# jizongFox/Self-paced-Contrastive-Learning

Measured on AMD Instinct MI355X. Metric: pretrain slices/sec/node (UNet+InfoNCE, 224^2, bs=32/GPU), higher is better.
Workload: dtype bf16; 1 GPU; BASELINE.json configs[1]: self-paced pretrain step, UNet base (max_channel=256) encoder to Conv5 + ProjectionHead(256,256,256) + SelfPacedSupConLoss(soft, partition labels, correct_grad) fwd+bwd + RAdam; slices_per_gpu=32, images_per_gpu_step=64, image=1x224x224, global_batch=32, parallelism=dp1, params=1311056, hipgraph=epocher, capture_steps=3

## Files before the change

include/spcl_hip.h:

```cpp
#ifndef SPCL_HIP_H
#define SPCL_HIP_H
#include <stddef.h>
#include <stdint.h>
#ifdef __cplusplus
extern "C" {
#endif

#define SPCL_F32 0
#define SPCL_BF16 1

#define SPCL_OK 0
#define SPCL_EINVAL (-1)
#define SPCL_ELAUNCH (-2)
#define SPCL_EUNSUPPORTED (-3)

#define SPCL_ABI_VERSION 28
int spcl_abi_version(void);
const char* spcl_last_error(void);

size_t spcl_supcon_workspace_bytes(int n, int d);
int spcl_supcon_forward(const float* z1, const float* z2, const float* labels, const float* mask, int n, int d,
                        float temperature, int sp_mode, float gamma, int correct_grad, float* ws, float* out,
                        void* stream);
int spcl_supcon_backward(const float* labels, const float* mask, int n, int d, float temperature, int sp_mode,
                         float gamma, const float* ws_fwd, float* ws_bwd, const float* out_fwd,
                         const float* grad_out, float* dz1, float* dz2, void* stream);
size_t spcl_supcon_bwd_workspace_bytes(int n, int d);
int spcl_supcon_unit_gradient_block(int n, int d, size_t* offset_floats, int* row_pitch);
int spcl_supcon_forward_heads(int K, const float* z1, const float* z2, size_t z_stride, const float* labels, int n,
                              int d, float temperature, int sp_mode, const float* gammas, int correct_grad, float* ws,
                              size_t ws_stride, float* out, void* stream);
int spcl_supcon_rows_supported(int n, int d);
int spcl_supcon_forward_rows(int K, const float* o1, const float* o2, size_t o_stride, const float* labels, int n, int d,
                             float temperature, int sp_mode, const float* gammas, int correct_grad, float* ws,
                             size_t ws_stride, float* out, void* stream);
int spcl_supcon_backward_heads(int K, const float* labels, int n, int d, float temperature, int sp_mode,
                               const float* gammas, const float* ws_fwd, size_t ws_stride, float* ws_bwd,
                               size_t wsb_stride, const float* out_fwd, const float* grad_out, float* dz1, float* dz2,
                               size_t z_stride, void* stream);
int spcl_supcon_materialize(const float* labels, const float* mask, int n, int d, float temperature, int sp_mode,
                            float gamma, const float* ws_fwd, float* sim_logits, float* sim_exp, float* pos_mask,
                            float* neg_mask, float* sp_mask, void* stream);

size_t spcl_supcon_xpos_workspace_bytes(int n, int d);
int spcl_supcon_xpos_forward(const float* z1, const float* z2, const float* labels, const float* mask, int n, int d,
                             float temperature, float* ws, float* out, void* stream);
int spcl_supcon_xpos_backward(const float* z1, const float* z2, int n, int d, float temperature, const float* ws,
                              const float* grad_out, float* dz1, float* dz2, void* stream);

// ... 107 lines not shown
int spcl_l2norm_rows_forward(const float* x, size_t rows, int O, float* z, void* stream);
int spcl_l2norm_rows_backward(const float* x, const float* dz, size_t rows, int O, float* dx, void* stream);

int spcl_group_l2norm_temp_forward(const float* l, size_t rows, long ld, int S, int K, int normalize, float T, float* z,
                                   void* stream);
int spcl_group_l2norm_temp_backward(const float* l, const float* dz, size_t rows, long ld, int S, int K, int normalize, float T,
                                    float* dl, void* stream);

#define SPCL_WGRAD_BATCH_MAX 16
typedef struct spcl_wgrad_item {
  const void* x;
  const void* dy;
  const float* in_scale;
  const float* in_shift;
  float* dw_oihw;
  int N, H, W, Cin, CinS, Cout, CoutS, in_mode;
  const void* x2;
  int x_up2;
} spcl_wgrad_item;
int spcl_conv_wgrad_batched_supported(int dtype, int Cin, int CinS, int Cout, int CoutS, int in_mode);
size_t spcl_conv_wgrad_batched_workspace_bytes(const spcl_wgrad_item* items, int n);
int spcl_conv3x3_wgrad_batched(const spcl_wgrad_item* items, int n, int accumulate, float* partial, void* stream);

#define SPCL_WGRAD_TAILS_MAX 16
typedef struct spcl_wgrad_tail {
  const float* partial;
  float* dw;
  int kind;
  int nsplit, nblk_ci, nblk_co, CIB, COB, Cin, Cout;
} spcl_wgrad_tail;
int spcl_wgrad_tail_capture(spcl_wgrad_tail* slot);
int spcl_conv3x3_wgrad_batched_tails(const spcl_wgrad_item* items, int n, const spcl_wgrad_tail* tails, int ntails,
                                     int accumulate, float* partial, void* stream);
int spcl_bn_finalize(float* stats, int ntiles, int C, int CS, const float* gamma, const float* beta,
                     float momentum, float eps, float* running_mean, float* running_var,
                     int64_t* num_batches_tracked, float* mean, float* invstd, float* scale, float* shift,
                     void* stream);
int spcl_bn_eval_affine(int C, int CS, const float* gamma, const float* beta, const float* running_mean,
                        const float* running_var, float eps, float* mean, float* invstd, float* scale, float* shift,
                        void* stream);
#define SPCL_BN_EVAL_MAX 32
typedef struct {
  const float* gamma;
  const float* beta;
  const float* running_mean;
  const float* running_var;
  float* st;
  int C, CS;
  float eps;
} spcl_bn_eval_item;
int spcl_bn_eval_affine_multi(const spcl_bn_eval_item* items, int n, void* stream);

int spcl_bnrelu_pool_forward(const void* y, int dtype, int N, int H, int W, int CS, const float* scale,
                             const float* shift, void* act_out, void* pool_out, void* stream);
size_t spcl_bnrelu_bwd_workspace_bytes(int N, int H, int W, int CS);
int spcl_bnrelu_pool_backward(const void* y, const void* dact, const void* dpool, int dtype, int N, int H, int W,
                              int C, int CS, const float* mean, const float* invstd, const float* scale,
                              const float* shift, int training, float* ws, float* dgamma, float* dbeta, void* dy,
                              void* stream);
int spcl_bnrelu_up2_forward(const void* y, int dtype, int N, int H, int W, int CS, const float* scale, const float* shift,
                            void* up_out, void* stream);
int spcl_bnrelu_pool_forward_strided(const void* y, int dtype, int N, int H, int W, int CS, const float* scale,
                                     const float* shift, void* act_out, int act_stride, void* pool_out, void* stream);
int spcl_bnrelu_pool_backward_strided(const void* y, const void* dact, int dact_stride, const void* dpool, int dtype, int N,
                                      int H, int W, int C, int CS, const float* mean, const float* invstd,
                                      const float* scale, const float* shift, int training, float* ws, float* dgamma,
// ... 328 lines not shown
```

self-paced-contrastive-learning_amd/csrc/wgrad.hip:

```cpp
#include <stdlib.h>
#include <vector>
#include "conv_common.hpp"

namespace spcl {

constexpr int WG_TW = 16, WG_HW = WG_TW + 2;

struct WgradArgs {
  const void* x;
  const void* x2;
  int xsplit;
  int x_up2;
  const void* dy;
  const float* in_scale;
  const float* in_shift;
  float* partial;
  int N, H, W, CinS, CinK, CoutS, in_mode;
  int tilesX, tilesY, ntiles, nblk_ci, nblk_co;
  int dbuf;
  int xcd_remap;
  unsigned long long* stamps;
};

template <typename T> __device__ __forceinline__ u32x4 wg_bnrelu_chunk(u32x4 raw, const float* sc, const float* sh);
template <> __device__ __forceinline__ u32x4 wg_bnrelu_chunk<float>(u32x4 raw, const float* s, const float* b) {
  f32x4 v = __builtin_bit_cast(f32x4, raw);
#pragma unroll
  for (int e = 0; e < 4; ++e) v[e] = fmaxf(fmaf(s[e], v[e], b[e]), 0.f);
  return __builtin_bit_cast(u32x4, v);
}
template <> __device__ __forceinline__ u32x4 wg_bnrelu_chunk<bf16_t>(u32x4 raw, const float* s, const float* b) {
  u32x4 out;
#pragma unroll
// ... 56 lines not shown
  static __device__ __forceinline__ int lane_col(int lane) { return Frag<bf16_t>::lane_col(lane); }
  static __device__ __forceinline__ int lane_chan_bytes(int lane) { return Frag<bf16_t>::lane_chan_bytes(lane); }
  static __device__ __forceinline__ type load(unsigned a0, int off, int pix_bytes, int plane_bytes) {
    type f;
    f.h = Frag<bf16_t>::load(a0, off, pix_bytes);
    f.m = Frag<bf16_t>::load(a0 + plane_bytes, off, pix_bytes);
    f.l = Frag<bf16_t>::load(a0 + 2 * plane_bytes, off, pix_bytes);
    return f;
  }
  static __device__ __forceinline__ f32x4 mfma(const type& a, const type& b, f32x4 c) {
    c = __builtin_amdgcn_mfma_f32_16x16x32_bf16(a.l, b.h, c, 0, 0, 0);
    c = __builtin_amdgcn_mfma_f32_16x16x32_bf16(a.h, b.l, c, 0, 0, 0);
    c = __builtin_amdgcn_mfma_f32_16x16x32_bf16(a.m, b.m, c, 0, 0, 0);
    c = __builtin_amdgcn_mfma_f32_16x16x32_bf16(a.m, b.h, c, 0, 0, 0);
    c = __builtin_amdgcn_mfma_f32_16x16x32_bf16(a.h, b.m, c, 0, 0, 0);
    c = __builtin_amdgcn_mfma_f32_16x16x32_bf16(a.h, b.h, c, 0, 0, 0);
    return c;
  }
  static constexpr int row_pad(int pix_bytes, int row_bytes) { return Frag<bf16_t>::row_pad(pix_bytes, row_bytes); }
};

#ifndef SPCL_WGRAD_STAMPS_BUILD
#define SPCL_WGRAD_STAMPS_BUILD 0
#endif
__device__ __forceinline__ void store_split(unsigned char* p, int plane_bytes, u32x4 v) {
  const Split3 a = split3_pair(__uint_as_float(v[0]), __uint_as_float(v[1]));
  const Split3 b = split3_pair(__uint_as_float(v[2]), __uint_as_float(v[3]));
  *(uint2*)p = make_uint2(a.hi, b.hi);
  *(uint2*)(p + plane_bytes) = make_uint2(a.mid, b.mid);
  *(uint2*)(p + 2 * plane_bytes) = make_uint2(a.lo, b.lo);
}

template <typename T, int MI, int NJ, int TH, int NWV, int IM>
__global__ __launch_bounds__(64 * NWV, 2) void conv3x3_wgrad_kernel(WgradArgs a) {
  constexpr int NTHR = 64 * NWV;
  constexpr int EPC = Chunk<T>::EPC;
  constexpr int LSZ = Frag<T>::LSZ, NPL = Frag<T>::PLANES, LCH = EPC * LSZ;
  constexpr int CIB = 16 * MI, COB = 16 * NJ;
  constexpr int XS = CIB * LSZ, DS = COB * LSZ;
  constexpr int XCP = CIB / EPC, DCP = COB / EPC;
  constexpr int XRP = WG_HW * XS + Frag<T>::row_pad(XS, WG_HW * XS);
  constexpr int DRP = WG_TW * DS + Frag<T>::row_pad(DS, WG_TW * DS);
  constexpr int NHROWS = TH + 2;
  constexpr int XPLB = NHROWS * XRP, DPLB = TH * DRP;
  constexpr int X_BYTES = NPL * XPLB, D_BYTES = NPL * DPLB, BUF_BYTES = X_BYTES + D_BYTES;
  constexpr int KSTEPS = TH * WG_TW / Frag<T>::KPIX;
  constexpr int XPL = NTHR / XCP, XRPI = XPL / WG_HW, NX = (NHROWS + XRPI - 1) / XRPI;
  constexpr int DPL = NTHR / DCP, DRPI = DPL / WG_TW, ND = (TH + DRPI - 1) / DRPI;
  static_assert(XRPI >= 1 && DRPI >= 1, "channel block too wide for the staging map");
  extern __shared__ __attribute__((aligned(16))) unsigned char lds[];
  const unsigned lds_base = (unsigned)(uintptr_t)(unsigned char __attribute__((address_space(3)))*)lds;

  const int lane = threadIdx.x & 63, wave = threadIdx.x >> 6;
  const int blk = blockIdx.y;
  const int bci = blk / a.nblk_co, bco = blk - bci * a.nblk_co;
  const int ci0 = bci * CIB, co0 = bco * COB;
  const int xch = threadIdx.x % XCP, xpl = threadIdx.x / XCP;
  const int xhy0 = xpl / WG_HW, xhx = xpl - xhy0 * WG_HW;
  const bool xact = xpl < XRPI * WG_HW;
  const int dch = threadIdx.x % DCP, dpl = threadIdx.x / DCP;
  const int dry0 = dpl / WG_TW, dcol = dpl - dry0 * WG_TW;
  float sc[EPC], sh[EPC];
  const bool bn_x2 = IM == 1 && a.x2 != nullptr;
  const bool bn_this = IM == 1 && (!bn_x2 || ci0 + xch * EPC >= a.xsplit);
  if (IM == 1) {
    const int cc = bn_x2 ? (bn_this ? ci0 + xch * EPC - a.xsplit : 0) : ci0 + xch * EPC;
#pragma unroll
    for (int e = 0; e < EPC; e += 4) {
      *(f32x4*)&sc[e] = *(const f32x4*)(a.in_scale + cc + e);
      *(f32x4*)&sh[e] = *(const f32x4*)(a.in_shift + cc + e);
    }
  }

  constexpr int NUNITS = 9 * MI, UPW = (NUNITS + NWV - 1) / NWV;
  f32x4 acc[UPW][NJ];
  int uoff[UPW];
#pragma unroll
  for (int uu = 0; uu < UPW; ++uu) {
    int u = wave + NWV * uu;
    if (u >= NUNITS) u = NUNITS - 1;
    const int tap = u / MI, m = u - tap * MI;
    const int ky = tap / 3, kx = tap - 3 * ky;
    uoff[uu] = ky * XRP + kx * XS + m * 16 * LSZ;
#pragma unroll
    for (int j = 0; j < NJ; ++j) acc[uu][j] = (f32x4){0.f, 0.f, 0.f, 0.f};
  }
  const unsigned xlane = (unsigned)(Frag<T>::lane_row(lane) * XRP + Frag<T>::lane_col(lane) * XS +
// ... 99 lines not shown
    constexpr bool K32 = Frag<T>::KPIX == 32;
    constexpr bool SKIP_DUP = NUNITS % NWV != 0;
    const bool last_real = wave + NWV * (UPW - 1) < NUNITS;
    auto kpos_x = [&](int ks) { return (K32 ? 2 * ks : ks / 4) * XRP + (K32 ? 0 : 4 * (ks % 4)) * XS; };
    auto kpos_d = [&](int ks) { return (K32 ? 2 * ks : ks / 4) * DRP + (K32 ? 0 : 4 * (ks % 4)) * DS; };
    typename Frag<T>::type bf[NJ], bf_next[NJ], af, af_next;
#pragma unroll
    for (int j = 0; j < NJ; ++j) bf[j] = Frag<T>::load(da0, kpos_d(0) + j * 16 * LSZ, DS, DPLB);
    af = Frag<T>::load(xa0 + uoff[0], kpos_x(0), XS, XPLB);
#pragma unroll
    for (int ks = 0; ks < KSTEPS; ++ks) {
#pragma unroll
      for (int uu = 0; uu < UPW; ++uu) {
        if (uu + 1 < UPW) af_next = Frag<T>::load(xa0 + uoff[uu + 1], kpos_x(ks), XS, XPLB);
        else if (ks + 1 < KSTEPS) {
          af_next = Frag<T>::load(xa0 + uoff[0], kpos_x(ks + 1), XS, XPLB);
#pragma unroll
          for (int j = 0; j < NJ; ++j) bf_next[j] = Frag<T>::load(da0, kpos_d(ks + 1) + j * 16 * LSZ, DS, DPLB);
        }
        if (!(SKIP_DUP && uu == UPW - 1 && !last_real)) {
#pragma unroll
          for (int j = 0; j < NJ; ++j) acc[uu][j] = Frag<T>::mfma(af, bf[j], acc[uu][j]);
        }
        af = af_next;
      }
#pragma unroll
      for (int j = 0; j < NJ; ++j) bf[j] = bf_next[j];
    }
  };

  unsigned long long t_store = 0, t_bar = 0, t_issue = 0, t_comp = 0, t_first = 0, t_all = 0, ntl = 0;
  const bool stamp = SPCL_WGRAD_STAMPS_BUILD && a.stamps != nullptr;
  const unsigned long long c_begin = stamp ? __builtin_amdgcn_s_memtime() : 0;
  const int G = (int)gridDim.x;
  const int pos = (a.xcd_remap && (G & 7) == 0) ? (int)(blockIdx.x & 7) * (G >> 3) + (int)(blockIdx.x >> 3) : (int)blockIdx.x;
  int tile = pos;
  int buf = 0;
  if (tile < a.ntiles) load_tile(tile);
  if (stamp) t_first = __builtin_amdgcn_s_memtime() - c_begin;
  while (tile < a.ntiles) {
    const unsigned long long c0 = stamp ? __builtin_amdgcn_s_memtime() : 0;
    store_tile(buf);
    const unsigned long long c1 = stamp ? __builtin_amdgcn_s_memtime() : 0;
    __syncthreads();
    const unsigned long long c2 = stamp ? __builtin_amdgcn_s_memtime() : 0;
    const int next = tile + gridDim.x;
    if (next < a.ntiles) load_tile(next);
    const unsigned long long c3 = stamp ? __builtin_amdgcn_s_memtime() : 0;
    compute_tile(buf);
    if (stamp) {
      t_store += c1 - c0; t_bar += c2 - c1; t_issue += c3 - c2; t_comp += __builtin_amdgcn_s_memtime() - c3;
      ++ntl;
    }
    if (a.dbuf) buf ^= 1;
    else __syncthreads();
    tile = next;
  }
  if (stamp) t_all = __builtin_amdgcn_s_memtime() - c_begin;

  const int r16 = lane & 15, g = lane >> 4;
  float* out = a.partial + ((size_t)blockIdx.x * gridDim.y + blk) * (9 * CIB * COB);
#pragma unroll
  for (int uu = 0; uu < UPW; ++uu) {
    const int u = wave + NWV * uu;
    if (u < NUNITS) {
      const int tap = u / MI, m = u - tap * MI;
#pragma unroll
      for (int j = 0; j < NJ; ++j)
#pragma unroll
        for (int r = 0; r < 4; ++r)
          out[(tap * CIB + m * 16 + 4 * g + r) * COB + j * 16 + r16] = acc[uu][j][r];
    }
  }
  if (stamp && threadIdx.x == 0) {
    unsigned long long* o = a.stamps + ((size_t)blockIdx.x * gridDim.y + blk) * 8;
    o[0] = t_first; o[1] = t_store; o[2] = t_bar; o[3] = t_issue; o[4] = t_comp; o[5] = t_all;
    o[6] = __builtin_amdgcn_s_memtime() - c_begin; o[7] = ntl;
  }
}

template <int VEC>
__global__ __launch_bounds__(1024) void wgrad_reduce_kernel(const float* __restrict__ partial, int nsplit, int nblk_ci,
                                                            int nblk_co, int CIB, int COB, int Cin, int Cout,
                                                            float* __restrict__ dw) {
  __shared__ float red[16][64 * VEC];
  const int nwaves = blockDim.x >> 6;
  const int lane = threadIdx.x & 63, wave = threadIdx.x >> 6;
  const int slab = 9 * CIB * COB;
  const int inner = (blockIdx.x * 64 + lane) * VEC;
  const int blk = blockIdx.y;
  const size_t nblk = (size_t)nblk_ci * nblk_co;
  float s[VEC];
#pragma unroll
  for (int e = 0; e < VEC; ++e) s[e] = 0.f;
  if (inner < slab) {
    const float* src = partial + (size_t)blk * slab + inner;
    const size_t stride = nblk * slab;
#pragma unroll 8
    for (int p = wave; p < nsplit; p += nwaves) {
      if (VEC == 4) {
        const f32x4 v = *(const f32x4*)(src + (size_t)p * stride);
#pragma unroll
        for (int e = 0; e < VEC; ++e) s[e] += v[e];
      } else {
        s[0] += src[(size_t)p * stride];
      }
    }
  }
#pragma unroll
  for (int e = 0; e < VEC; ++e) red[wave][lane * VEC + e] = s[e];
// ... 211 lines not shown
  {
    const double px = (double)N * H * W, es = dtype == SPCL_F32 ? 4.0 : 2.0;
    prof_cost(px * ((in_mode == 2 ? CinS * 4.0 : CinK * es) + CoutS * es) + 9.0 * Cin * Cout * 4.0,
              2.0 * px * 9.0 * Cin * Cout);
  }
  if (dtype == SPCL_F32 && split) launch_wgrad_t<split_f32>(a, p, st);
  else if (dtype == SPCL_F32) launch_wgrad_t<float>(a, p, st);
  else if (dtype == SPCL_BF16) launch_wgrad_t<bf16_t>(a, p, st);
  else {
    set_error("conv3x3_wgrad: dtype %d", dtype);
    return SPCL_EINVAL;
  }
  if (tail != nullptr) {
    tail->partial = partial; tail->dw = dw_oihw; tail->kind = 0; tail->nsplit = p.nsplit; tail->nblk_ci = p.nblk_ci;
    tail->nblk_co = p.nblk_co; tail->CIB = 16 * p.MI; tail->COB = 16 * p.NJ; tail->Cin = Cin; tail->Cout = Cout;
  } else {
    launch_wgrad_reduce(partial, p.nsplit, p.nblk_ci, p.nblk_co, 16 * p.MI, 16 * p.NJ, Cin, Cout, dw_oihw, st);
  }
  if (a.stamps) {
    std::vector<unsigned long long> h(nwg * 8);
    (void)hipStreamSynchronize(st);
    (void)hipMemcpy(h.data(), a.stamps, h.size() * 8, hipMemcpyDeviceToHost);
    double s[8] = {0};
    for (size_t i = 0; i < nwg; ++i)
      for (int k = 0; k < 8; ++k) s[k] += (double)h[i * 8 + k];
    for (int k = 0; k < 8; ++k) s[k] /= (double)nwg;
    fprintf(stderr, "[wgrad stamps] %dx%d Cin%d Cout%d MI%d NJ%d TH%d wgs=%zu tiles/wg=%.1f | memtime ticks per wg: first-load "
            "issue %.0f, store %.0f, barrier %.0f, next-load issue %.0f, compute %.0f, loop total %.0f, with epilogue %.0f\n",
            H, W, Cin, Cout, p.MI, p.NJ, p.TH, nwg, s[7], s[0], s[1], s[2], s[3], s[4], s[5], s[6]);
  }
  SPCL_LAUNCH_CHECK("conv3x3_wgrad");
  return SPCL_OK;
}
```

self-paced-contrastive-learning_amd/functional.py:

```python
from __future__ import annotations

import ctypes
import math
import os
from ctypes import c_double, c_float, c_int

import torch

from . import native as _n

SP_NONE, SP_HARD, SP_SOFT = 0, 1, 2


def take_grad_sink(param, needed: bool = True):
    if not needed or param is None:
        return None
    sink = getattr(param, "_grad_sink", None)
    if sink is None or not getattr(param, "_grad_sink_armed", False):
        return None
    if sink.shape != param.shape or sink.dtype != torch.float32 or not sink.is_contiguous() or sink.device != param.device:
        return None
    param._grad_sink_armed = False
    return sink

# ... 1121 lines not shown
    if want_rows and stats_acc is None:
        nt = _n.call("spcl_conv_stat_rows", dt_code, N, H, W, cin_k, cout_s)
        rows = torch.empty(_n.call("spcl_bn_stats_elems", nt, cout_s), dtype=torch.float32, device=dev)
        rows.ntiles = nt
    _n.call("spcl_conv3x3_forward_acc", _n.ptr(x_store), dt_code, N, H, W, cin_k, cout_s, _n.ptr(wp),
            ctypes.byref(in_bn) if in_bn is not None else None, _n.ptr(in_scale), _n.ptr(in_shift), _n.ptr(y),
            _n.ptr(stats_acc), _n.ptr(rows), _n.stream())
    return y, rows


def _bn_stats(stats, cfg: BlockCfg, C, cs, gamma, beta, which, dev):
    st = torch.empty(4, cs, dtype=torch.float32, device=dev)
    g, b = gamma.detach().contiguous().float(), beta.detach().contiguous().float()
    rm, rv, nbt = cfg.buffers[which]
    if cfg.training:
        upd = cfg.track[which]
        _n.call("spcl_bn_finalize", _n.ptr(stats), stats.ntiles, C, cs, _n.ptr(g), _n.ptr(b), c_float(cfg.momentum),
                c_float(cfg.eps), _n.ptr(rm if upd else None), _n.ptr(rv if upd else None),
                _n.ptr(nbt if upd else None), _n.ptr(st[0]), _n.ptr(st[1]), _n.ptr(st[2]), _n.ptr(st[3]), _n.stream())
    else:
        pre = _EVAL_AFFINE.pop((rm.data_ptr(), cs), None) if rm.dtype == torch.float32 else None
        if pre is not None:
            return pre
        _n.call("spcl_bn_eval_affine", C, cs, _n.ptr(g), _n.ptr(b), _n.ptr(rm), _n.ptr(rv), c_float(cfg.eps),
                _n.ptr(st[0]), _n.ptr(st[1]), _n.ptr(st[2]), _n.ptr(st[3]), _n.stream())
    return st


class DeferredWgrads:

    def __init__(self):
        self.items, self.keep, self.targets = [], [], set()
        self.tails = []

    def add(self, x_store, dy, scale, shift, sink, N, H, W, cin, cin_s, cout, cout_s, in_mode, x2=None, x_up2=False):
        it = _n.WgradItem(x_store.data_ptr(), dy.data_ptr(), scale.data_ptr() if scale is not None else None,
                          shift.data_ptr() if shift is not None else None, sink.data_ptr(), N, H, W, cin, cin_s, cout,
                          cout_s, in_mode, x2.data_ptr() if x2 is not None else None, 1 if x_up2 else 0)
        self.items.append(it)
        self.keep.append((x_store, dy, scale, shift, x2))
        self.targets.add(sink.data_ptr())
        if len(self.items) == _QUEUE_MAX[0]:
            self.flush()

    def capture_tail(self, sink, keep, launch):
        tail = _n.WgradTail()
        _n.call("spcl_wgrad_tail_capture", ctypes.byref(tail))
        try:
            launch()
        finally:
            _n.call("spcl_wgrad_tail_capture", None)
        if tail.kind < 0:
            return False
        self.tails.append(tail)
        self.keep.append(keep)
        self.targets.add(sink.data_ptr())
        if len(self.tails) == _QUEUE_MAX[1]:
            self.flush()
        return True

    def flush(self):
        if not self.items and not self.tails:
            return
        wgrad_batched(self.items, accumulate=False, device=self.keep[0][1].device, tails=self.tails)
        self.items, self.keep, self.tails = [], [], []


_QUEUE_MAX = (min(_n.WGRAD_BATCH_MAX, int(os.environ.get("SPCL_WGRAD_QUEUE_MAX", _n.WGRAD_BATCH_MAX))),
              min(_n.WGRAD_TAILS_MAX, int(os.environ.get("SPCL_WGRAD_QUEUE_MAX", _n.WGRAD_TAILS_MAX))))
_CONV_UP2 = os.environ.get("SPCL_CONV_UP2", "1") != "0"
_UP2_BWD_FUSED = os.environ.get("SPCL_UP2_BWD_FUSED", "1") != "0"
_CONV_SPLIT = os.environ.get("SPCL_CONV_SPLIT", "1") != "0"
_CONV_CAT = os.environ.get("SPCL_CONV_CAT", "1") != "0"
_PACK_AT = os.environ.get("SPCL_PACK_AT", "1") != "0"
_ACC_FILL = os.environ.get("SPCL_ACC_FILL", "1") != "0"
_GAP = os.environ.get("SPCL_GAP", "1") != "0"
_TAILS = os.environ.get("SPCL_WGRAD_TAILS", "1") != "0"


def sink_queue(sink):
    return getattr(sink, "_spcl_queue", None) if sink is not None else None


def wgrad_batched(items, accumulate, device, tails=()):
    arr, ws = None, None
    if items:
        arr = (_n.WgradItem * len(items))(*items)
        nbytes = _n.call("spcl_conv_wgrad_batched_workspace_bytes", arr, len(items))
        if nbytes == 0:
            raise RuntimeError("wgrad_batched: unsupported item (bf16 NHWC, channel counts multiples of 64, in_mode 0/1)")
        ws = torch.empty(nbytes // 4, dtype=torch.float32, device=device)
    tarr = (_n.WgradTail * len(tails))(*tails) if tails else None
    _n.call("spcl_conv3x3_wgrad_batched_tails", arr, len(items), tarr, len(tails), int(bool(accumulate)), _n.ptr(ws),
            _n.stream())


def _wgrad(x_store, dy, dt_code, N, H, W, cin, cin_s, cin_k, cout, cout_s, in_mode, scale, shift, sink=None):
    dev = dy.device
    queue = sink_queue(sink)
    if (queue is not None and cin_s == cin_k
            and _n.call("spcl_conv_wgrad_batched_supported", dt_code, cin, cin_s, cout, cout_s, in_mode)):
        queue.add(x_store, dy, scale, shift, sink, N, H, W, cin, cin_s, cout, cout_s, in_mode)
        return None
    nbytes = _n.call("spcl_conv_wgrad_workspace_bytes", N, H, W, cin_k, cout_s)
    ws = torch.empty(nbytes // 4, dtype=torch.float32, device=dev)
    dw = _grad_buffer(sink, (cout, cin, 3, 3), dev)

    def launch():
        _n.call("spcl_conv3x3_wgrad", _n.ptr(x_store), _n.ptr(dy), dt_code, N, H, W, cin, cin_s, cin_k, cout, cout_s,
                in_mode, _n.ptr(scale), _n.ptr(shift), _n.ptr(ws), _n.ptr(dw), _n.stream())

    if queue is not None and _TAILS:
        if queue.capture_tail(sink, (ws, dy, x_store, scale, shift), launch):
            return None
        return dw
    launch()
    return dw


def _wgrad_up2(x_half, dy, dt_code, N, H, W, cin, cout, cout_s, sink=None):
    dev = dy.device
    queue = sink_queue(sink)
    if queue is not None and _n.call("spcl_conv_wgrad_batched_supported", dt_code, cin, cin, cout, cout_s, 0):
        queue.add(x_half, dy, None, None, sink, N, H, W, cin, cin, cout, cout_s, 0, x_up2=True)
        return None
    nbytes = _n.call("spcl_conv_wgrad_workspace_bytes", N, H, W, cin, cout_s)
    ws = torch.empty(nbytes // 4, dtype=torch.float32, device=dev)
    dw = _grad_buffer(sink, (cout, cin, 3, 3), dev)

    def launch():
        _n.call("spcl_conv3x3_wgrad_up2", _n.ptr(x_half), _n.ptr(dy), dt_code, N, H, W, cin, cout, cout_s, _n.ptr(ws),
                _n.ptr(dw), _n.stream())

    if queue is not None and _TAILS:
        if queue.capture_tail(sink, (ws, dy, x_half), launch):
# ... 2233 lines not shown
```

self-paced-contrastive-learning_amd/native.py:

```python
from __future__ import annotations

import ctypes
import os
from ctypes import c_char_p, c_double, c_float, c_int, c_long, c_size_t, c_void_p

import torch

HERE = os.path.dirname(os.path.abspath(__file__))
LIB_PATH = os.path.join(HERE, "lib", "libspcl_hip.so")
SPCL_F32, SPCL_BF16 = 0, 1

_lib = None

_P = c_void_p
_SIGNATURES = {
    "spcl_abi_version": (c_int, []),
    "spcl_last_error": (c_char_p, []),
    "spcl_supcon_workspace_bytes": (c_size_t, [c_int, c_int]),
    "spcl_supcon_forward": (c_int, [_P, _P, _P, _P, c_int, c_int, c_float, c_int, c_float, c_int, _P, _P, _P]),
    "spcl_supcon_backward": (c_int, [_P, _P, c_int, c_int, c_float, c_int, c_float, _P, _P, _P, _P, _P, _P, _P]),
    "spcl_supcon_bwd_workspace_bytes": (c_size_t, [c_int, c_int]),
    "spcl_supcon_unit_gradient_block": (c_int, [c_int, c_int, _P, _P]),
    "spcl_supcon_materialize": (c_int, [_P, _P, c_int, c_int, c_float, c_int, c_float, _P, _P, _P, _P, _P, _P, _P]),
    "spcl_supcon_xpos_workspace_bytes": (c_size_t, [c_int, c_int]),
# ... 31 lines not shown
    "spcl_conv_pack_weights_multi_zero": (c_int, [_P, c_int, c_int, _P, c_int, c_int, c_int, _P, _P, c_size_t, _P]),
    "spcl_conv_num_tiles": (c_int, [c_int, c_int, c_int]),
    "spcl_conv_stat_rows": (c_int, [c_int, c_int, c_int, c_int, c_int, c_int]),
    "spcl_conv_set_gemm": (None, [c_int]),
    "spcl_conv_set_f32_split": (None, [c_int]),
    "spcl_conv_get_f32_split": (c_int, []),
    "spcl_conv_cat_supported": (c_int, [c_int, c_int, c_int, c_int, c_int, c_int]),
    "spcl_conv3x3_forward_cat": (c_int, [_P, _P, c_int, c_int, c_int, c_int, c_int, c_int, _P, _P, _P, _P, _P, _P]),
    "spcl_conv_split_supported": (c_int, [c_int, c_int, c_int, c_int, c_int, c_int]),
    "spcl_conv3x3_forward_split": (c_int, [_P, c_int, c_int, c_int, c_int, c_int, c_int, _P, _P, _P, _P]),
    "spcl_conv_split_bnstats_supported": (c_int, [c_int, c_int, c_int, c_int, c_int, c_int]),
    "spcl_conv3x3_dgrad_split_bnstats": (c_int, [_P, c_int, c_int, c_int, c_int, c_int, c_int, _P, _P, _P, _P, _P, _P, _P, _P,
                                                 _P]),
    "spcl_conv_up2_supported": (c_int, [c_int, c_int, c_int, c_int, c_int, c_int]),
    "spcl_conv3x3_forward_up2": (c_int, [_P, c_int, c_int, c_int, c_int, c_int, c_int, _P, _P, _P, _P]),
    "spcl_conv3x3_wgrad_up2": (c_int, [_P, _P, c_int, c_int, c_int, c_int, c_int, c_int, c_int, _P, _P, _P]),
    "spcl_conv3x3_wgrad_cat": (c_int, [_P, _P, _P, c_int, c_int, c_int, c_int, c_int, c_int, c_int, _P, _P, _P, _P, _P]),
    "spcl_bn_stats_elems": (c_size_t, [c_int, c_int]),
    "spcl_conv3x3_forward": (c_int, [_P, c_int, c_int, c_int, c_int, c_int, c_int, c_int, _P, c_int, _P, _P, _P, _P,
                                     _P]),
    "spcl_supcon_forward_heads": (c_int, [c_int, _P, _P, c_size_t, _P, c_int, c_int, c_float, c_int, _P, c_int, _P,
                                          c_size_t, _P, _P]),
    "spcl_supcon_rows_supported": (c_int, [c_int, c_int]),
    "spcl_supcon_forward_rows": (c_int, [c_int, _P, _P, c_size_t, _P, c_int, c_int, c_float, c_int, _P, c_int, _P,
                                         c_size_t, _P, _P]),
    "spcl_supcon_backward_heads": (c_int, [c_int, _P, c_int, c_int, c_float, c_int, _P, _P, c_size_t, _P, c_size_t, _P,
                                           _P, _P, _P, c_size_t, _P]),
    "spcl_conv_wgrad_workspace_bytes": (c_size_t, [c_int, c_int, c_int, c_int, c_int]),
    "spcl_conv3x3_wgrad": (c_int, [_P, _P, c_int, c_int, c_int, c_int, c_int, c_int, c_int, c_int, c_int, c_int, _P,
                                   _P, _P, _P, _P]),
    "spcl_conv_wgrad_batched_supported": (c_int, [c_int, c_int, c_int, c_int, c_int, c_int]),
    "spcl_conv_wgrad_batched_workspace_bytes": (c_size_t, [_P, c_int]),
    "spcl_conv3x3_wgrad_batched": (c_int, [_P, c_int, c_int, _P, _P]),
    "spcl_wgrad_tail_capture": (c_int, [_P]),
    "spcl_conv3x3_wgrad_batched_tails": (c_int, [_P, c_int, _P, c_int, c_int, _P, _P]),
    "spcl_bn_finalize": (c_int, [_P, c_int, c_int, c_int, _P, _P, c_float, c_float, _P, _P, _P, _P, _P, _P, _P, _P]),
    "spcl_bn_eval_affine": (c_int, [c_int, c_int, _P, _P, _P, _P, c_float, _P, _P, _P, _P, _P]),
    "spcl_bn_eval_affine_multi": (c_int, [_P, c_int, _P]),
    "spcl_bnrelu_pool_forward": (c_int, [_P, c_int, c_int, c_int, c_int, c_int, _P, _P, _P, _P, _P]),
    "spcl_bnrelu_up2_forward": (c_int, [_P, c_int, c_int, c_int, c_int, c_int, _P, _P, _P, _P]),
    "spcl_bnrelu_pool_forward_strided": (c_int, [_P, c_int, c_int, c_int, c_int, c_int, _P, _P, _P, c_int, _P, _P]),
    "spcl_bnrelu_pool_backward_strided": (c_int, [_P, _P, c_int, _P, c_int, c_int, c_int, c_int, c_int, c_int, _P, _P, _P,
                                                  _P, c_int, _P, _P, _P, _P, _P]),
    "spcl_bnrelu_bwd_workspace_bytes": (c_size_t, [c_int, c_int, c_int, c_int]),
    "spcl_bnrelu_pool_backward": (c_int, [_P, _P, _P, c_int, c_int, c_int, c_int, c_int, c_int, _P, _P, _P, _P,
                                          c_int, _P, _P, _P, _P, _P]),
    "spcl_bnrelu_backward_up2": (c_int, [_P, _P, _P, c_int, c_int, c_int, c_int, c_int, c_int, _P, _P, _P, _P, c_int, _P, _P, _P, _P,
                                         _P]),
    "spcl_bnrelu_backward_bcast": (c_int, [_P, _P, c_int, c_int, c_int, c_int, c_int, c_int, _P, _P, _P, _P, c_int, _P, _P,
                                           _P, _P, _P]),
    "spcl_bnrelu_image_wgrad_workspace_bytes": (c_size_t, [c_int, c_int, c_int, c_int]),
    "spcl_bnrelu_backward_image_wgrad": (c_int, [_P, _P, _P, c_int, c_int, c_int, c_int, c_int, c_int, _P, _P, _P, _P,
                                                 c_int, _P, _P, _P, _P, _P]),
    "spcl_accumulate_scalars": (c_int, [c_int, _P, _P, _P, _P]),
    "spcl_stage_bytes": (c_int, [_P, _P, c_size_t, _P]),
    "spcl_conv_dgrad_bnstats_supported": (c_int, [c_int, c_int, c_int, c_int, c_int, c_int]),
    "spcl_conv3x3_dgrad_bnstats": (c_int, [_P, c_int, c_int, c_int, c_int, c_int, c_int, _P, _P, _P, _P, _P, _P, _P, _P]),
    "spcl_conv_dgrad_poolstats_supported": (c_int, [c_int, c_int, c_int, c_int, c_int, c_int, c_int, c_int]),
    "spcl_conv3x3_dgrad_poolstats": (c_int, [_P, c_int, c_int, c_int, c_int, c_int, c_int, _P, _P, _P, c_int, c_int, _P, _P,
                                             _P, _P, _P]),
    "spcl_bnrelu_pool_backward_rows": (c_int, [_P, _P, _P, c_int, c_int, c_int, c_int, c_int, c_int, c_int, _P, _P, _P, _P,
                                               c_int, _P, _P, _P, _P, _P]),
    "spcl_bnrelu_backward_rows": (c_int, [_P, _P, _P, _P, c_int, c_int, c_int, c_int, c_int, c_int, c_int, _P, _P, _P, _P,
                                          c_int, _P, _P, _P, _P, _P, _P]),
    "spcl_image_autocorr_rows": (c_int, [c_int, c_int, c_int]),
    "spcl_image_autocorr": (c_int, [_P, c_int, c_int, c_int, _P, _P]),
# ... 160 lines not shown
class WgradItem(ctypes.Structure):
    _fields_ = [("x", c_void_p), ("dy", c_void_p), ("in_scale", c_void_p), ("in_shift", c_void_p),
                ("dw_oihw", c_void_p), ("N", c_int), ("H", c_int), ("W", c_int), ("Cin", c_int), ("CinS", c_int),
                ("Cout", c_int), ("CoutS", c_int), ("in_mode", c_int), ("x2", c_void_p), ("x_up2", c_int)]


class PackItem(ctypes.Structure):
    _fields_ = [("w_oihw", c_void_p), ("fwd", c_void_p), ("dgrad", c_void_p), ("Cin", c_int), ("Cout", c_int),
                ("H", c_int), ("W", c_int)]


BN_EVAL_MAX = 32


class BnEvalItem(ctypes.Structure):
    _fields_ = [("gamma", c_void_p), ("beta", c_void_p), ("running_mean", c_void_p), ("running_var", c_void_p),
                ("st", c_void_p), ("C", c_int), ("CS", c_int), ("eps", c_float)]


class BnAcc(ctypes.Structure):
    _fields_ = [("acc", c_void_p), ("gamma", c_void_p), ("beta", c_void_p), ("running_mean", c_void_p),
                ("running_var", c_void_p), ("num_batches_tracked", c_void_p), ("st", c_void_p), ("momentum", c_float),
                ("eps", c_float), ("count", c_float), ("C", c_int), ("CS", c_int)]


PACK_MULTI_MAX = 24


class WgradTail(ctypes.Structure):
    _fields_ = [("partial", c_void_p), ("dw", c_void_p), ("kind", c_int), ("nsplit", c_int), ("nblk_ci", c_int),
                ("nblk_co", c_int), ("CIB", c_int), ("COB", c_int), ("Cin", c_int), ("Cout", c_int)]


ABI_VERSION = 28
WGRAD_BATCH_MAX = 16
WGRAD_TAILS_MAX = 16
_NO_STATUS = ("spcl_abi_version", "spcl_block1_recompute_supported", "spcl_block1_kernels_take", "spcl_conv16_bwd_fused_image_supported", "spcl_conv3x3_forward_image_acorr_rows", "spcl_image_autocorr_rows", "spcl_conv_dgrad_bnstats_image_supported", "spcl_conv16_bwd_fused_supported", "spcl_conv16_bwd_fused_splits", "spcl_conv_num_tiles", "spcl_conv_stat_rows", "spcl_conv_set_gemm", "spcl_conv_set_f32_split", "spcl_conv_get_f32_split", "spcl_supcon_unit_gradient_block", "spcl_conv_cat_supported", "spcl_conv_up2_supported", "spcl_conv_split_supported", "spcl_conv_split_bnstats_supported", "spcl_conv1x1_bwd_rows", "spcl_profile_count", "spcl_conv_dgrad_bnstats_supported", "spcl_conv_dgrad_poolstats_supported",
              "spcl_conv_wgrad_batched_supported", "spcl_conv_bn_acc_supported", "spcl_conv_dgrad_bnstats_acc_supported",
              "spcl_conv_dgrad_poolstats_acc_supported", "spcl_supcon_rows_supported", "spcl_bnrelu_gap_supported",
              "spcl_conv_dgrad_poolmax_supported", "spcl_conv_dgrad_poolmax_acc_supported",
              "spcl_conv16_bwd_fused_image_pooled_supported")


class NativeLibraryError(RuntimeError):
    pass


def lib():
    global _lib
    if _lib is None:
        if not os.path.exists(LIB_PATH):
            raise NativeLibraryError(
                f"{LIB_PATH} is missing: build it with `python self-paced-contrastive-learning_amd/build.py` "
                "(there is no CPU / eager fallback for the hot path)")
        L = ctypes.CDLL(LIB_PATH)
        L.spcl_abi_version.restype, L.spcl_abi_version.argtypes = c_int, []
        have = L.spcl_abi_version()
        if have != ABI_VERSION:
            raise NativeLibraryError(
                f"{LIB_PATH} has C-ABI version {have}, this binding was written for {ABI_VERSION} (include/spcl_hip.h "
                "SPCL_ABI_VERSION): a stale build -- rebuild with `python self-paced-contrastive-learning_amd/build.py`")
        for name, (res, args) in _SIGNATURES.items():
            fn = getattr(L, name, None)
            if fn is None:
                continue
            fn.restype, fn.argtypes = res, args
        _lib = L
    return _lib


def call(name: str, *args):
# ... 38 lines not shown
```

Baseline: 32270 slices/s.

## Batch narrow-channel conv wgrads into one load-balanced grouped kernel launch

Measured after the change: 32490 slices/s (median of 6 runs). No clear change (+0.7%).

```diff
diff --git a/include/spcl_hip.h b/include/spcl_hip.h
--- a/include/spcl_hip.h
+++ b/include/spcl_hip.h
@@ -14,7 +14,7 @@
 #define SPCL_ELAUNCH (-2)
 #define SPCL_EUNSUPPORTED (-3)
 
-#define SPCL_ABI_VERSION 28
+#define SPCL_ABI_VERSION 29
 int spcl_abi_version(void);
 const char* spcl_last_error(void);
 
@@ -188,6 +188,11 @@
 int spcl_wgrad_tail_capture(spcl_wgrad_tail* slot);
 int spcl_conv3x3_wgrad_batched_tails(const spcl_wgrad_item* items, int n, const spcl_wgrad_tail* tails, int ntails,
                                      int accumulate, float* partial, void* stream);
+#define SPCL_WGRAD_NARROW_MAX 16
+int spcl_conv_wgrad_narrow_batched_supported(int dtype, int Cin, int CinS, int Cout, int CoutS, int in_mode);
+size_t spcl_conv_wgrad_narrow_batched_workspace_bytes(const spcl_wgrad_item* items, int n);
+int spcl_conv3x3_wgrad_narrow_batched(const spcl_wgrad_item* items, int n, float* partial, spcl_wgrad_tail* tails_out,
+                                      void* stream);
 int spcl_bn_finalize(float* stats, int ntiles, int C, int CS, const float* gamma, const float* beta,
                      float momentum, float eps, float* running_mean, float* running_var,
                      int64_t* num_batches_tracked, float* mean, float* invstd, float* scale, float* shift,
diff --git a/self-paced-contrastive-learning_amd/csrc/wgrad.hip b/self-paced-contrastive-learning_amd/csrc/wgrad.hip
--- a/self-paced-contrastive-learning_amd/csrc/wgrad.hip
+++ b/self-paced-contrastive-learning_amd/csrc/wgrad.hip
@@ -1,4 +1,5 @@
 #include <stdlib.h>
+#include <string.h>
 #include <vector>
 #include "conv_common.hpp"
 
@@ -121,7 +122,7 @@
 }
 
 template <typename T, int MI, int NJ, int TH, int NWV, int IM>
-__global__ __launch_bounds__(64 * NWV, 2) void conv3x3_wgrad_kernel(WgradArgs a) {
+__device__ __forceinline__ void wgrad_body(const WgradArgs& a, const int pos, const int G, const int blk, const int slab) {
   constexpr int NTHR = 64 * NWV;
   constexpr int EPC = Chunk<T>::EPC;
   constexpr int LSZ = Frag<T>::LSZ, NPL = Frag<T>::PLANES, LCH = EPC * LSZ;
@@ -141,7 +142,6 @@
   const unsigned lds_base = (unsigned)(uintptr_t)(unsigned char __attribute__((address_space(3)))*)lds;
 
   const int lane = threadIdx.x & 63, wave = threadIdx.x >> 6;
-  const int blk = blockIdx.y;
   const int bci = blk / a.nblk_co, bco = blk - bci * a.nblk_co;
   const int ci0 = bci * CIB, co0 = bco * COB;
   const int xch = threadIdx.x % XCP, xpl = threadIdx.x / XCP;
@@ -307,8 +307,6 @@
   unsigned long long t_store = 0, t_bar = 0, t_issue = 0, t_comp = 0, t_first = 0, t_all = 0, ntl = 0;
   const bool stamp = SPCL_WGRAD_STAMPS_BUILD && a.stamps != nullptr;
   const unsigned long long c_begin = stamp ? __builtin_amdgcn_s_memtime() : 0;
-  const int G = (int)gridDim.x;
-  const int pos = (a.xcd_remap && (G & 7) == 0) ? (int)(blockIdx.x & 7) * (G >> 3) + (int)(blockIdx.x >> 3) : (int)blockIdx.x;
   int tile = pos;
   int buf = 0;
   if (tile < a.ntiles) load_tile(tile);
@@ -319,7 +317,7 @@
     const unsigned long long c1 = stamp ? __builtin_amdgcn_s_memtime() : 0;
     __syncthreads();
     const unsigned long long c2 = stamp ? __builtin_amdgcn_s_memtime() : 0;
-    const int next = tile + gridDim.x;
+    const int next = tile + G;
     if (next < a.ntiles) load_tile(next);
     const unsigned long long c3 = stamp ? __builtin_amdgcn_s_memtime() : 0;
     compute_tile(buf);
@@ -334,7 +332,7 @@
   if (stamp) t_all = __builtin_amdgcn_s_memtime() - c_begin;
 
   const int r16 = lane & 15, g = lane >> 4;
-  float* out = a.partial + ((size_t)blockIdx.x * gridDim.y + blk) * (9 * CIB * COB);
+  float* out = a.partial + (size_t)slab * (9 * CIB * COB);
 #pragma unroll
   for (int uu = 0; uu < UPW; ++uu) {
     const int u = wave + NWV * uu;
@@ -348,9 +346,46 @@
     }
   }
   if (stamp && threadIdx.x == 0) {
-    unsigned long long* o = a.stamps + ((size_t)blockIdx.x * gridDim.y + blk) * 8;
+    unsigned long long* o = a.stamps + (size_t)slab * 8;
     o[0] = t_first; o[1] = t_store; o[2] = t_bar; o[3] = t_issue; o[4] = t_comp; o[5] = t_all;
     o[6] = __builtin_amdgcn_s_memtime() - c_begin; o[7] = ntl;
+  }
+}
+
+template <typename T, int MI, int NJ, int TH, int NWV, int IM>
+__global__ __launch_bounds__(64 * NWV, 2) void conv3x3_wgrad_kernel(WgradArgs a) {
+  const int G = (int)gridDim.x;
+  const int pos = (a.xcd_remap && (G & 7) == 0) ? (int)(blockIdx.x & 7) * (G >> 3) + (int)(blockIdx.x >> 3) : (int)blockIdx.x;
+  wgrad_body<T, MI, NJ, TH, NWV, IM>(a, pos, G, (int)blockIdx.y, (int)(blockIdx.x * gridDim.y + blockIdx.y));
+}
+
+constexpr int WN_MAX = SPCL_WGRAD_NARROW_MAX;
+struct WnArgs {
+  WgradArgs it[WN_MAX];
+  int wg0[WN_MAX];
+  int nsplit[WN_MAX];
+  int kind[WN_MAX];
+  int n;
+};
+__global__ __launch_bounds__(512, 4) void conv3x3_wgrad_narrow_kernel(WnArgs q) {
+  const int wg = (int)blockIdx.x;
+  int idx = 0;
+#pragma unroll 1
+  for (int i = 1; i < q.n; ++i)
+    if (wg >= q.wg0[i]) idx = i;
+  const WgradArgs& a = q.it[idx];
+  const int ns = q.nsplit[idx], local = wg - q.wg0[idx];
+  const int blk = local / ns, split = local - blk * ns;
+  const int slab = split * (a.nblk_ci * a.nblk_co) + blk;
+  switch (q.kind[idx]) {
+    case 0: wgrad_body<bf16_t, 1, 2, 14, 8, 0>(a, split, ns, blk, slab); break;
+    case 1: wgrad_body<bf16_t, 1, 2, 14, 8, 1>(a, split, ns, blk, slab); break;
+    case 2: wgrad_body<bf16_t, 1, 2, 16, 8, 0>(a, split, ns, blk, slab); break;
+    case 3: wgrad_body<bf16_t, 1, 2, 16, 8, 1>(a, split, ns, blk, slab); break;
+    case 4: wgrad_body<bf16_t, 2, 2, 14, 8, 0>(a, split, ns, blk, slab); break;
+    case 5: wgrad_body<bf16_t, 2, 2, 14, 8, 1>(a, split, ns, blk, slab); break;
+    case 6: wgrad_body<bf16_t, 2, 2, 16, 8, 0>(a, split, ns, blk, slab); break;
+    default: wgrad_body<bf16_t, 2, 2, 16, 8, 1>(a, split, ns, blk, slab); break;
   }
 }
 
@@ -628,3 +663,136 @@
   SPCL_LAUNCH_CHECK("conv3x3_wgrad");
   return SPCL_OK;
 }
+
+namespace spcl {
+
+static bool wn_shape_ok(int dtype, int Cin, int CinS, int Cout, int CoutS, int in_mode) {
+  return dtype == SPCL_BF16 && (Cin == 16 || Cin == 32) && CinS == Cin && (Cout == 32 || Cout == 64) && CoutS == Cout &&
+         (in_mode == 0 || in_mode == 1);
+}
+
+static bool wn_item_ok(const spcl_wgrad_item& s) {
+  return s.x && s.dy && s.dw_oihw && s.N > 0 && s.H > 0 && s.W > 0 &&
+         wn_shape_ok(SPCL_BF16, s.Cin, s.CinS, s.Cout, s.CoutS, s.in_mode) && (s.in_mode == 0 || (s.in_scale && s.in_shift)) &&
+         s.x2 == nullptr && s.x_up2 == 0 && (uintptr_t)s.x % 16 == 0 && (uintptr_t)s.dy % 16 == 0 &&
+         (long)s.N * s.H * s.W * (s.CinS > s.CoutS ? s.CinS : s.CoutS) < (1L << 31);
+}
+
+struct WnPlan {
+  WnArgs args;
+  WgradPlan lp[WN_MAX];
+  size_t off[WN_MAX];
+  size_t floats;
+  int nwg;
+  size_t lds;
+};
+
+static void wn_plan(const spcl_wgrad_item* items, int n, WnPlan& pl) {
+  long work[WN_MAX];
+  pl.lds = 0;
+  int used = 0;
+  for (int i = 0; i < n; ++i) {
+    const spcl_wgrad_item& s = items[i];
+    WgradPlan& p = pl.lp[i];
+    p = wgrad_plan(s.N, s.H, s.W, s.Cin, s.CoutS, 2);
+    const size_t lds = 2 * wgrad_lds_bytes(p.MI, p.NJ, p.TH, 2);
+    if (lds > pl.lds) pl.lds = lds;
+    work[i] = (long)wgrad_lds_bytes(p.MI, p.NJ, p.TH, 2);
+    pl.args.nsplit[i] = 1;
+    used += p.nblk_ci * p.nblk_co;
+  }
+  int per_cu = (int)((160 * 1024) / pl.lds);
+  if (per_cu > 2) per_cu = 2;
+  const int P = 256 * per_cu;
+  auto len = [&](int i) { return (long)cdiv(pl.lp[i].ntiles, pl.args.nsplit[i]) * work[i]; };
+  for (;;) {
+    int longest = 0;
+    for (int i = 1; i < n; ++i)
+      if (len(i) > len(longest)) longest = i;
+    const int nblk = pl.lp[longest].nblk_ci * pl.lp[longest].nblk_co;
+    if (pl.args.nsplit[longest] >= pl.lp[longest].ntiles || used + nblk > P) break;
+    pl.args.nsplit[longest] += 1;
+    used += nblk;
+  }
+  long longest = 0;
+  for (int i = 0; i < n; ++i)
+    if (len(i) > longest) longest = len(i);
+  int wg = 0;
+  pl.floats = 0;
+  for (int i = 0; i < n; ++i) {
+    const WgradPlan& p = pl.lp[i];
+    const int per_wg = (int)(longest / work[i]);
+    pl.args.nsplit[i] = cdiv(p.ntiles, per_wg);
+    pl.args.wg0[i] = wg;
+    pl.args.kind[i] = 4 * (p.MI - 1) + 2 * (p.TH == 16 ? 1 : 0) + items[i].in_mode;
+    pl.off[i] = pl.floats;
+    const int nblk = p.nblk_ci * p.nblk_co;
+    wg += nblk * pl.args.nsplit[i];
+    pl.floats += (size_t)nblk * pl.args.nsplit[i] * 9 * (16 * p.MI) * (16 * p.NJ);
+  }
+  pl.nwg = wg;
+  pl.args.n = n;
+}
+
+}
+
+extern "C" int spcl_conv_wgrad_narrow_batched_supported(int dtype, int Cin, int CinS, int Cout, int CoutS, int in_mode) {
+  return wn_shape_ok(dtype, Cin, CinS, Cout, CoutS, in_mode) ? 1 : 0;
+}
+
+extern "C" size_t spcl_conv_wgrad_narrow_batched_workspace_bytes(const spcl_wgrad_item* items, int n) {
+  if (!items || n < 1 || n > WN_MAX) return 0;
+  for (int i = 0; i < n; ++i)
+    if (!wn_item_ok(items[i])) return 0;
+  WnPlan pl;
+  wn_plan(items, n, pl);
+  return pl.floats * sizeof(float);
+}
+
+extern "C" int spcl_conv3x3_wgrad_narrow_batched(const spcl_wgrad_item* items, int n, float* partial,
+                                                 spcl_wgrad_tail* tails_out, void* stream) {
+  SPCL_CHECK_ARG(n >= 1 && n <= WN_MAX, "conv3x3_wgrad_narrow_batched: %d items (1..%d)", n, WN_MAX);
+  SPCL_CHECK_ARG(items && partial && (uintptr_t)partial % 16 == 0, "conv3x3_wgrad_narrow_batched: null or misaligned pointer");
+  for (int i = 0; i < n; ++i)
+    SPCL_CHECK_ARG(wn_item_ok(items[i]), "conv3x3_wgrad_narrow_batched: item %d: bf16 NHWC, 16 / 32 -> 32 / 64 channels, dense, "
+                                         "in_mode 0/1 (with scale/shift)", i);
+  WnPlan pl;
+  wn_plan(items, n, pl);
+  hipStream_t st = (hipStream_t)stream;
+  double bytes = 0.0, flops = 0.0;
+  for (int i = 0; i < n; ++i) {
+    const spcl_wgrad_item& s = items[i];
+    const WgradPlan& p = pl.lp[i];
+    WgradArgs& a = pl.args.it[i];
+    a.x = s.x; a.x2 = nullptr; a.xsplit = 0; a.x_up2 = 0; a.dy = s.dy; a.in_scale = s.in_scale; a.in_shift = s.in_shift;
+    a.partial = partial + pl.off[i];
+    a.N = s.N; a.H = s.H; a.W = s.W; a.CinS = s.CinS; a.CinK = s.Cin; a.CoutS = s.CoutS; a.in_mode = s.in_mode;
+    a.tilesX = p.tilesX; a.tilesY = p.tilesY; a.ntiles = p.ntiles; a.nblk_ci = p.nblk_ci; a.nblk_co = p.nblk_co;
+    a.dbuf = 1; a.xcd_remap = 0; a.stamps = nullptr;
+    const double px = (double)s.N * s.H * s.W;
+    bytes += px * (s.Cin + s.Cout) * 2.0 + 9.0 * s.Cin * s.Cout * 4.0;
+    flops += 2.0 * px * 9.0 * s.Cin * s.Cout;
+  }
+  for (int i = n; i < WN_MAX; ++i) {
+    memset(&pl.args.it[i], 0, sizeof(WgradArgs));
+    pl.args.wg0[i] = pl.nwg; pl.args.nsplit[i] = 1; pl.args.kind[i] = 0;
+  }
+  prof_cost(bytes, flops);
+  if (pl.lds > 65536)
+    spcl::func_lds_limit((const void*)conv3x3_wgrad_narrow_kernel, (int)pl.lds, "conv3x3_wgrad_narrow_kernel");
+  SPCL_LAUNCH(conv3x3_wgrad_narrow_kernel, dim3(pl.nwg), dim3(512), pl.lds, st, pl.args);
+  for (int i = 0; i < n; ++i) {
+    const WgradPlan& p = pl.lp[i];
+    if (tails_out != nullptr) {
+      spcl_wgrad_tail& t = tails_out[i];
+      t.partial = partial + pl.off[i]; t.dw = items[i].dw_oihw; t.kind = 0; t.nsplit = pl.args.nsplit[i];
+      t.nblk_ci = p.nblk_ci; t.nblk_co = p.nblk_co; t.CIB = 16 * p.MI; t.COB = 16 * p.NJ; t.Cin = items[i].Cin;
+      t.Cout = items[i].Cout;
+    } else {
+      launch_wgrad_reduce(partial + pl.off[i], pl.args.nsplit[i], p.nblk_ci, p.nblk_co, 16 * p.MI, 16 * p.NJ, items[i].Cin,
+                          items[i].Cout, items[i].dw_oihw, st);
+    }
+  }
+  SPCL_LAUNCH_CHECK("conv3x3_wgrad_narrow_batched");
+  return SPCL_OK;
+}
diff --git a/self-paced-contrastive-learning_amd/functional.py b/self-paced-contrastive-learning_amd/functional.py
--- a/self-paced-contrastive-learning_amd/functional.py
+++ b/self-paced-contrastive-learning_amd/functional.py
@@ -1177,6 +1177,7 @@
     def __init__(self):
         self.items, self.keep, self.targets = [], [], set()
         self.tails = []
+        self.narrow = []
 
     def add(self, x_store, dy, scale, shift, sink, N, H, W, cin, cin_s, cout, cout_s, in_mode, x2=None, x_up2=False):
         it = _n.WgradItem(x_store.data_ptr(), dy.data_ptr(), scale.data_ptr() if scale is not None else None,
@@ -1187,6 +1188,15 @@
         self.targets.add(sink.data_ptr())
         if len(self.items) == _QUEUE_MAX[0]:
             self.flush()
+
+    def add_narrow(self, x_store, dy, scale, shift, sink, N, H, W, cin, cout, in_mode):
+        if len(self.narrow) == _n.WGRAD_NARROW_MAX or len(self.tails) + len(self.narrow) >= _QUEUE_MAX[1]:
+            self.flush()
+        self.narrow.append(_n.WgradItem(x_store.data_ptr(), dy.data_ptr(), scale.data_ptr() if scale is not None else None,
+                                        shift.data_ptr() if shift is not None else None, sink.data_ptr(), N, H, W, cin,
+                                        cin, cout, cout, in_mode, None, 0))
+        self.keep.append((x_store, dy, scale, shift))
+        self.targets.add(sink.data_ptr())
 
     def capture_tail(self, sink, keep, launch):
         tail = _n.WgradTail()
@@ -1200,14 +1210,30 @@
         self.tails.append(tail)
         self.keep.append(keep)
         self.targets.add(sink.data_ptr())
-        if len(self.tails) == _QUEUE_MAX[1]:
+        if len(self.tails) + len(self.narrow) >= _QUEUE_MAX[1]:
             self.flush()
         return True
 
+    def launch_narrow(self):
+        if not self.narrow:
+            return
+        n = len(self.narrow)
+        arr, out = (_n.WgradItem * n)(*self.narrow), (_n.WgradTail * n)()
+        nbytes = _n.call("spcl_conv_wgrad_narrow_batched_workspace_bytes", arr, n)
+        if nbytes == 0:
+            raise RuntimeError("wgrad narrow batched: unsupported item (bf16 NHWC, 16 / 32 -> 32 / 64 channels, in_mode 0/1)")
+        ws = torch.empty(nbytes // 4, dtype=torch.float32, device=self.keep[0][1].device)
+        _n.call("spcl_conv3x3_wgrad_narrow_batched", arr, n, _n.ptr(ws), out, _n.stream())
+        self.tails += list(out)
+        self.keep.append((ws,))
+        self.narrow = []
+
     def flush(self):
-        if not self.items and not self.tails:
+        if not self.items and not self.tails and not self.narrow:
             return
-        wgrad_batched(self.items, accumulate=False, device=self.keep[0][1].device, tails=self.tails)
+        device = self.keep[0][1].device
+        self.launch_narrow()
+        wgrad_batched(self.items, accumulate=False, device=device, tails=self.tails)
         self.items, self.keep, self.tails = [], [], []
 
 
@@ -1221,6 +1247,7 @@
 _ACC_FILL = os.environ.get("SPCL_ACC_FILL", "1") != "0"
 _GAP = os.environ.get("SPCL_GAP", "1") != "0"
 _TAILS = os.environ.get("SPCL_WGRAD_TAILS", "1") != "0"
+_WGRAD_NARROW_BATCHED = os.environ.get("SPCL_WGRAD_NARROW_BATCHED", "1") != "0"
 
 
 def sink_queue(sink):
@@ -1246,6 +1273,11 @@
     if (queue is not None and cin_s == cin_k
             and _n.call("spcl_conv_wgrad_batched_supported", dt_code, cin, cin_s, cout, cout_s, in_mode)):
         queue.add(x_store, dy, scale, shift, sink, N, H, W, cin, cin_s, cout, cout_s, in_mode)
+        return None
+    if (queue is not None and _TAILS and _WGRAD_NARROW_BATCHED and cin_s == cin_k and x_store.data_ptr() % 16 == 0
+            and dy.data_ptr() % 16 == 0
+            and _n.call("spcl_conv_wgrad_narrow_batched_supported", dt_code, cin, cin_s, cout, cout_s, in_mode)):
+        queue.add_narrow(x_store, dy, scale, shift, sink, N, H, W, cin, cout, in_mode)
         return None
     nbytes = _n.call("spcl_conv_wgrad_workspace_bytes", N, H, W, cin_k, cout_s)
     ws = torch.empty(nbytes // 4, dtype=torch.float32, device=dev)
diff --git a/self-paced-contrastive-learning_amd/native.py b/self-paced-contrastive-learning_amd/native.py
--- a/self-paced-contrastive-learning_amd/native.py
+++ b/self-paced-contrastive-learning_amd/native.py
@@ -87,6 +87,9 @@
     "spcl_conv_wgrad_batched_supported": (c_int, [c_int, c_int, c_int, c_int, c_int, c_int]),
     "spcl_conv_wgrad_batched_workspace_bytes": (c_size_t, [_P, c_int]),
     "spcl_conv3x3_wgrad_batched": (c_int, [_P, c_int, c_int, _P, _P]),
+    "spcl_conv_wgrad_narrow_batched_supported": (c_int, [c_int, c_int, c_int, c_int, c_int, c_int]),
+    "spcl_conv_wgrad_narrow_batched_workspace_bytes": (c_size_t, [_P, c_int]),
+    "spcl_conv3x3_wgrad_narrow_batched": (c_int, [_P, c_int, _P, _P, _P]),
     "spcl_wgrad_tail_capture": (c_int, [_P]),
     "spcl_conv3x3_wgrad_batched_tails": (c_int, [_P, c_int, _P, c_int, c_int, _P, _P]),
     "spcl_bn_finalize": (c_int, [_P, c_int, c_int, c_int, _P, _P, c_float, c_float, _P, _P, _P, _P, _P, _P, _P, _P]),
@@ -313,11 +316,12 @@
                 ("nblk_co", c_int), ("CIB", c_int), ("COB", c_int), ("Cin", c_int), ("Cout", c_int)]
 
 
-ABI_VERSION = 28
+ABI_VERSION = 29
 WGRAD_BATCH_MAX = 16
 WGRAD_TAILS_MAX = 16
+WGRAD_NARROW_MAX = 16
 _NO_STATUS = ("spcl_abi_version", "spcl_block1_recompute_supported", "spcl_block1_kernels_take", "spcl_conv16_bwd_fused_image_supported", "spcl_conv3x3_forward_image_acorr_rows", "spcl_image_autocorr_rows", "spcl_conv_dgrad_bnstats_image_supported", "spcl_conv16_bwd_fused_supported", "spcl_conv16_bwd_fused_splits", "spcl_conv_num_tiles", "spcl_conv_stat_rows", "spcl_conv_set_gemm", "spcl_conv_set_f32_split", "spcl_conv_get_f32_split", "spcl_supcon_unit_gradient_block", "spcl_conv_cat_supported", "spcl_conv_up2_supported", "spcl_conv_split_supported", "spcl_conv_split_bnstats_supported", "spcl_conv1x1_bwd_rows", "spcl_profile_count", "spcl_conv_dgrad_bnstats_supported", "spcl_conv_dgrad_poolstats_supported",
-              "spcl_conv_wgrad_batched_supported", "spcl_conv_bn_acc_supported", "spcl_conv_dgrad_bnstats_acc_supported",
+              "spcl_conv_wgrad_batched_supported", "spcl_conv_wgrad_narrow_batched_supported", "spcl_conv_bn_acc_supported", "spcl_conv_dgrad_bnstats_acc_supported",
               "spcl_conv_dgrad_poolstats_acc_supported", "spcl_supcon_rows_supported", "spcl_bnrelu_gap_supported",
               "spcl_conv_dgrad_poolmax_supported", "spcl_conv_dgrad_poolmax_acc_supported",
               "spcl_conv16_bwd_fused_image_pooled_supported")
```
